# hzi-bifo/RiboDetector

Measured on AMD Instinct MI355X. Metric: reads/sec classified, 100 bp paired-end, higher is better.
Workload: dtype f16x3-split (f32 accumulate); 1 GPU; BASELINE configs[2]: paired-end 100 bp, --ensure rrna, 1048576 pairs/step/GPU x 49 steps (51.4 M total); pinned host bytes -> H2D -> kernels -> labels D2H (SURVEY 8d region ii); read_len=100, ensure=rrna, kernel_variant=mfma_f16x3_t32, parallelism=reads sharded x1, label gather to rank 0, rccl_ranks=1, forced_dist=False, prefix_k=12

## Files before the change

include/ribodetector_amd.h:

```cpp
#ifndef RIBODETECTOR_AMD_H
#define RIBODETECTOR_AMD_H

#include <stddef.h>
#include <stdint.h>

#ifndef RD_API
#define RD_API __attribute__((visibility("default")))
#endif

#ifdef __cplusplus
extern "C" {
#endif

#define RD_OK 0
#define RD_E_INVALID (-1)
#define RD_E_HIP (-2)
#define RD_E_UNSUPPORTED (-3)
#define RD_E_WORKSPACE (-4)

#define RD_ENSURE_NONE 0
#define RD_ENSURE_RRNA 1
#define RD_ENSURE_NORRNA 2
#define RD_ENSURE_BOTH 3

// ... 30 lines not shown
RD_API int rd_sync_results(rd_model *m, void *stream);
RD_API int rd_refine(const rd_model *m, const uint8_t *arena, const int64_t *seq_off, const int32_t *seq_len, int64_t n,
              int32_t max_len, float *logits, uint8_t *labels, const float *mate_logits, float thresh, void *stream);

#define RD_PREFIX_K_MIN 4
#define RD_PREFIX_K_MAX 13
RD_API size_t rd_prefix_table_bytes(int32_t k);
RD_API size_t rd_prefix_scratch_bytes(int32_t k);
RD_API int rd_set_prefix_table(rd_model *m, int32_t k, void *table, size_t table_bytes, void *scratch, size_t scratch_bytes, void *stream);
RD_API int rd_prefix_k(const rd_model *m);

RD_API size_t rd_classify_workspace_bytes(int64_t n, int32_t max_len);

RD_API int rd_classify(const rd_model *m, const uint8_t *arena, const int64_t *seq_off, const int32_t *seq_len, int64_t n,
                int32_t max_len, float *logits, uint8_t *labels, void *workspace, size_t workspace_bytes, void *stream);

RD_API int rd_pair_fuse(const float *logits1, const float *logits2, int64_t n, int32_t ensure_mode, int8_t *pair_labels,
                 uint64_t *counts, void *stream);

RD_API int rd_count_labels(const uint8_t *labels, int64_t n, uint64_t *counts, void *stream);

RD_API int rd_encode_codes(const uint8_t *arena, const int64_t *seq_off, const int32_t *seq_len, int64_t n, int32_t max_len,
                    int32_t stride, uint8_t *codes, void *stream);

RD_API int rd_encode_onehot_padded(const uint8_t *arena, const int64_t *seq_off, const int32_t *seq_len, int64_t n,
                            int32_t max_len, float *onehot, void *stream);

RD_API int rd_pack_plan(const int32_t *seq_len, int64_t n, int32_t max_len, int64_t *sorted_idx, int64_t *unsorted_idx,
                 int64_t *batch_sizes, int64_t *total_steps, void *workspace, size_t workspace_bytes, void *stream);
RD_API int rd_pack_onehot(const uint8_t *arena, const int64_t *seq_off, const int32_t *seq_len, int64_t n, int32_t max_len,
// ... 121 lines not shown
```

ribodetector_amd/_native.py:

```python
import ctypes as C
import os

_HERE = os.path.dirname(os.path.abspath(__file__))
LIB_PATH = os.environ.get("RD_HIP_LIB") or os.path.join(_HERE, "csrc", "librd_hip.so")

ENSURE_MODES = {"none": 0, "rrna": 1, "norrna": 2, "both": 3}
SEMANTICS = {"packed": 0, "gpu": 0, "padded": 1, "cpu": 1}
PREFIX_K_MIN, PREFIX_K_MAX, PREFIX_K_AUTO = 4, 13, 12
VARIANTS = {"auto": 0, "mfma_f32": 1, "simple": 2, "mfma_f16x3_t32": 4}
DIAG_VARIANTS = {"mfma_f32_a0s0": 10, "mfma_f32_a1s0": 11, "mfma_f32_a0s1": 12, "mfma_f32_a1s1": 13,
                 "mfma_f32_diag_noew": 20, "mfma_f32_diag_nomfma": 21, "mfma_f32_diag_mfmaonly": 22, "mfma_f32_diag_mfmabar": 23}
if os.path.basename(LIB_PATH).startswith("librd_hip_diag"):
    VARIANTS = dict(VARIANTS, **DIAG_VARIANTS)

SYMBOLS = [
    "rd_model_create", "rd_model_destroy", "rd_set_variant", "rd_variant_available", "rd_set_semantics", "rd_set_refine", "rd_set_refine_async", "rd_sync_results", "rd_refine", "rd_prefix_table_bytes", "rd_prefix_scratch_bytes", "rd_set_prefix_table", "rd_prefix_k", "rd_classify_workspace_bytes", "rd_classify",
    "rd_pair_fuse", "rd_count_labels", "rd_encode_codes", "rd_encode_onehot_padded", "rd_pack_plan",
    "rd_pack_onehot", "rd_profile_enable", "rd_profile_read", "rd_last_error", "rd_version",
    "rd_gz_workspace_bytes", "rd_gz_out_bound", "rd_gz_compress_selected", "rd_gz_eof_block", "rd_gz_inflate_members",
    "rd_fastq_index_workspace_bytes", "rd_fastq_index", "rd_fastq_gather", "rd_fastq_sample", "rd_fastq_strip_mark", "rd_fasta_index_workspace_bytes", "rd_fasta_index", "rd_fasta_gather", "rd_fasta_sample", "rd_select_workspace_bytes", "rd_select_pack", "rd_stream_create", "rd_stream_destroy", "rd_copy_bytes", "rd_gz_stream_workspace_bytes", "rd_gz_stream_inflate",
    "rd_gz_range_workspace_bytes", "rd_gz_range_decode", "rd_gz_range_resolve_workspace_bytes", "rd_gz_range_resolve",
    "rd_report_workspace_bytes", "rd_report_out_bound", "rd_report_format",
    "rd_pair_split", "rd_pair_expand_labels",
]
LABEL_SKIP = 2


class RdWeights(C.Structure):
    _fields_ = [(n, C.POINTER(C.c_float)) for n in
                ("w_ih", "w_hh", "b_ih", "b_hh", "w_ih_r", "w_hh_r", "b_ih_r", "b_hh_r", "w_out", "b_out")] + \
               [("input_size", C.c_int32), ("hidden_size", C.c_int32), ("num_classes", C.c_int32)]
# ... 21 lines not shown
    L.rd_variant_available.argtypes = [C.c_int]
    L.rd_set_semantics.argtypes = [vp, C.c_int]
    L.rd_set_refine.argtypes = [vp, C.c_float]
    L.rd_set_refine_async.argtypes = [vp, C.c_int]
    L.rd_sync_results.argtypes = [vp, vp]
    L.rd_refine.argtypes = [vp, vp, vp, vp, i64, i32, vp, vp, vp, C.c_float, vp]
    L.rd_prefix_table_bytes.argtypes = [i32]
    L.rd_prefix_table_bytes.restype = sz
    L.rd_prefix_scratch_bytes.argtypes = [i32]
    L.rd_prefix_scratch_bytes.restype = sz
    L.rd_set_prefix_table.argtypes = [vp, i32, vp, sz, vp, sz, vp]
    L.rd_prefix_k.argtypes = [vp]
    L.rd_classify_workspace_bytes.argtypes = [i64, i32]
    L.rd_classify_workspace_bytes.restype = sz
    L.rd_classify.argtypes = [vp, vp, vp, vp, i64, i32, vp, vp, vp, sz, vp]
    L.rd_pair_fuse.argtypes = [vp, vp, i64, i32, vp, vp, vp]
    L.rd_count_labels.argtypes = [vp, i64, vp, vp]
    L.rd_encode_codes.argtypes = [vp, vp, vp, i64, i32, i32, vp, vp]
    L.rd_encode_onehot_padded.argtypes = [vp, vp, vp, i64, i32, vp, vp]
    L.rd_pack_plan.argtypes = [vp, i64, i32, vp, vp, vp, vp, vp, sz, vp]
    L.rd_pack_onehot.argtypes = [vp, vp, vp, i64, i32, vp, vp, vp, vp]
    L.rd_gz_workspace_bytes.argtypes = [i64, i64]
    L.rd_gz_workspace_bytes.restype = sz
    L.rd_gz_out_bound.argtypes = [i64]
    L.rd_gz_out_bound.restype = sz
    L.rd_gz_compress_selected.argtypes = [vp, i64, vp, vp, i64, i32, vp, sz, vp, vp, sz, vp]
    L.rd_gz_eof_block.argtypes = [vp, sz]
    L.rd_gz_inflate_members.argtypes = [vp, i64, vp, i64, vp, i64, vp, vp]
    L.rd_fastq_index_workspace_bytes.argtypes = [i64]
    L.rd_fastq_index_workspace_bytes.restype = sz
# ... 132 lines not shown
```

ribodetector_amd/csrc/rd_kernels.hip:

```cpp
#include <stdlib.h>
#include "rd_common.hpp"
#include "rd_prep.hpp"
#include "rd_recurrence.hpp"
#include "rd_sort.hpp"
#include "rd_lstm_f32.hpp"
#include "rd_lstm_t32.hpp"
#include "rd_refine.hpp"
#include "rd_encode.hpp"
#include "rd_deflate.hpp"
#include "rd_inflate_dev.hpp"
#include "rd_inflate_stream.hpp"
#include "rd_fastq_index.hpp"
#include "rd_fasta_index.hpp"
#include "rd_report.hpp"
#include "rd_pairs.hpp"

extern "C" {

const char *rd_last_error(void) { return g_err; }
const char *rd_version(void) { return "ribodetector_amd 0.1.0 (gfx950)"; }

int rd_model_create(const rd_weights *w, int device, rd_model **out) {
    if (!w || !out) RD_FAIL(RD_E_INVALID, "rd_model_create: null argument");
    if (w->input_size != 4 || w->hidden_size != HID || w->num_classes != 2)
// ... 284 lines not shown
        m->prof_launches_accum += 1;
    }
    m->prof_count = 0;
    return RD_OK;
}

int rd_profile_read(rd_model *m, int64_t *launches, double *total_ms) {
    if (!m) RD_FAIL(RD_E_INVALID, "rd_profile_read: null model");
    int rc = rd_profile_drain(m);
    if (rc) return rc;
    if (launches) *launches = m->prof_launches_accum;
    if (total_ms) *total_ms = m->prof_ms_accum;
    return RD_OK;
}

int rd_classify(const rd_model *cm, const uint8_t *arena, const int64_t *seq_off, const int32_t *seq_len, int64_t n,
                int32_t max_len, float *logits, uint8_t *labels, void *workspace, size_t workspace_bytes, void *stream) {
    rd_model *m = const_cast<rd_model *>(cm);
    if (!m || !logits) RD_FAIL(RD_E_INVALID, "rd_classify: null model or logits");
    if (n < 0 || n > 0x7fffffffLL) RD_FAIL(RD_E_INVALID, "rd_classify: n=%lld out of range", (long long)n);
    if (max_len < 1 || max_len > MAX_LEN_LIMIT) RD_FAIL(RD_E_INVALID, "rd_classify: max_len=%d out of range [1,%d]", max_len, MAX_LEN_LIMIT);
    if (n == 0) return RD_OK;
    if (!arena || !seq_off || !seq_len || !workspace) RD_FAIL(RD_E_INVALID, "rd_classify: null input pointer");
    hipStream_t st = (hipStream_t)stream;
    const SortPlan sp = sort_plan(n, max_len);
    if (workspace_bytes < sp.total) RD_FAIL(RD_E_WORKSPACE, "workspace too small: %zu < %zu", workspace_bytes, sp.total);
    bool deferred = false;
    int join_after_launch = -1;
    if (m->refine_async && m->refine_thresh > 0.0f) {
        hipStreamCaptureStatus cap = hipStreamCaptureStatusNone;
        (void)hipStreamIsCapturing(st, &cap);
        deferred = cap == hipStreamCaptureStatusNone;
    }
    if (deferred) {
        bool clash = false;
        for (int x = 0; x < 2 && !clash; ++x)
            for (int k = 0; k < m->q_npend[x] && !clash; ++k) {
                const auto &pd = m->q_pend[x][k];
                const char *lo = (const char *)pd.p[3], *la = (const char *)pd.p[4];
                clash = (m->semantics == RD_SEM_PADDED && pd.max_len != max_len) ||
                        arena == pd.p[0] || seq_off == pd.p[1] || seq_len == pd.p[2] ||
                        ((const char *)logits < lo + 8 * pd.n && lo < (const char *)logits + 8 * n) ||
                        (labels && la && (const char *)labels < la + pd.n && la < (const char *)labels + n);
            }
        if (clash) { int rc0 = rd_sync_results(m, stream); if (rc0) return rc0; }
        if (m->q_calls >= m->refine_async) {
            const int old = m->q_cur;
            int rc0 = rd_async_flush(m, st, old);
            if (rc0) return rc0;
            m->q_cur ^= 1;
            m->q_calls = 0;
            rc0 = rd_async_join(m, st, m->q_cur);
            if (rc0) return rc0;
            join_after_launch = old;
        }
        int rc1 = rd_async_acquire(m, st, m->q_cur);
        if (rc1) return rc1;
    }
    if (m->semantics == RD_SEM_PADDED && m->rev_tab_len != max_len) {
        hipLaunchKernelGGL(rd_revtab_kernel, dim3(1), dim3(512), 0, st, m->d, max_len);
        m->rev_tab_len = max_len;
    }
    int32_t *steps = nullptr, *order = nullptr, *pfx = nullptr;
    const int pk = m->variant == m->ptab_variant ? m->prefix_k : 0;
    int rc = run_steps_and_buckets(arena, seq_off, seq_len, n, max_len, m->semantics, workspace, workspace_bytes, steps, order, pk, pfx, st);
    if (rc) return rc;
    ReadBatch rb{arena, seq_off, seq_len, steps, order, n, max_len, m->semantics, m->d.rev_tab, pk > 0 ? m->ptab : m->d.zero_row, pfx, pk,
                 deferred ? rd_queue(m, m->q_cur) : RefineQueue{nullptr, nullptr, 0}, m->refine_thresh};
    hipEvent_t *ev = nullptr;
    if (m->prof_enabled) {
        if (m->prof_count == 512) { rc = rd_profile_drain(m); if (rc) return rc; }
        ev = &m->prof_ev[2 * m->prof_count];
        for (int i = 0; i < 2; ++i)
            if (!ev[i]) RD_HIP(hipEventCreate(&ev[i]));
        RD_HIP(hipEventRecord(ev[0], st));
    }
    if (m->variant == RD_VARIANT_SIMPLE) {
        const int64_t nwg = (n + SB - 1) / SB;
        hipLaunchKernelGGL(rd_lstm_simple_kernel, dim3((unsigned)nwg), dim3(512), 0, st, m->d, rb, logits, labels);
    } else {
        const int64_t nwg = (n + BT - 1) / BT;
        const dim3 grid((unsigned)nwg), blk(256);
        switch (m->variant) {
// ... 14 lines not shown
    }
    RD_HIP(hipGetLastError());
    if (ev) { RD_HIP(hipEventRecord(ev[1], st)); m->prof_count++; }
    if (join_after_launch >= 0) {
        rc = rd_async_join(m, st, join_after_launch);
        if (rc) return rc;
    }
    if (m->refine_thresh > 0.0f) {
        if (!deferred) return rd_refine_launch(m, rb, logits, labels, nullptr, m->refine_thresh, st);
        auto &pd = m->q_pend[m->q_cur][m->q_npend[m->q_cur]++];
        pd.p[0] = arena; pd.p[1] = seq_off; pd.p[2] = seq_len; pd.p[3] = logits; pd.p[4] = labels;
        pd.n = n; pd.max_len = max_len; pd.sem = m->semantics; pd.thresh = m->refine_thresh;
        m->q_calls++;
    }
    return RD_OK;
}

int rd_pair_fuse(const float *logits1, const float *logits2, int64_t n, int32_t ensure_mode, int8_t *pair_labels,
                 uint64_t *counts, void *stream) {
    if (n < 0 || ensure_mode < 0 || ensure_mode > 3) RD_FAIL(RD_E_INVALID, "rd_pair_fuse: bad n or ensure_mode");
    if (n == 0) return RD_OK;
    if (!logits1 || !logits2 || !pair_labels) RD_FAIL(RD_E_INVALID, "rd_pair_fuse: null pointer");
    int64_t nb = (n + 2047) / 2048;
    if (nb > 1024) nb = 1024;
    const bool vec = (((uintptr_t)logits1 | (uintptr_t)logits2) & 15) == 0 && ((uintptr_t)pair_labels & 1) == 0;
    if (vec)
        hipLaunchKernelGGL(rd_pair_fuse_kernel<true>, dim3((unsigned)nb), dim3(256), 0, (hipStream_t)stream, (const float2 *)logits1,
                           (const float2 *)logits2, n, ensure_mode, pair_labels, counts);
    else
        hipLaunchKernelGGL(rd_pair_fuse_kernel<false>, dim3((unsigned)nb), dim3(256), 0, (hipStream_t)stream, (const float2 *)logits1,
// ... 559 lines not shown
```

ribodetector_amd/csrc/rd_lstm_f32.hpp:

```cpp
#pragma once
#include "rd_recurrence.hpp"

namespace {

struct __attribute__((aligned(16))) LstmSmem {
    float Hs[NT][16][HSTR];
    float Hl[NT][16][HSTR];
    f32x4 cA[NT][256];
    f32x4 cB[NT][256];
    f32x4 lut[5][4][16][2];
    float wout[2][HID];
    float dummy[256];
    uint8_t codes[2][TC][BT];
    int T[BT];
    int Lr[BT];
    long long off[BT];
    int orig[BT];
    int k0[BT];
    int prow[BT];
    int tmax;
};

__device__ __forceinline__ void rd_f32_load_h(LstmSmem &S, const uint8_t *ptab, int read) {
    const int piece = threadIdx.x & 3;
// ... 37 lines not shown
template <int ACT>
__device__ __forceinline__ float act_tanh(float x) {
    if (ACT == 0) return rd_tanh(x);
    return __builtin_fmaf(-2.0f, __builtin_amdgcn_rcpf(1.0f + __builtin_amdgcn_exp2f(x * 2.88539008177792681f)), 1.0f);
}

template <int ACT, int SCHED, int DIAG = 0, bool BUILD = false>
__global__ __launch_bounds__(256, 1) void rd_lstm_mfma_f32_kernel(DevModel d, ReadBatch rb, float *__restrict__ logits,
                                                                  uint8_t *__restrict__ labels) {
    __shared__ LstmSmem S;
    const int tid = threadIdx.x, lane = tid & 63;
    const int wave = __builtin_amdgcn_readfirstlane(tid >> 6);
    const int q = lane >> 4, l15 = lane & 15;

    const int nz = BUILD ? 0 : (rb.pk > 0 ? 1 << (2 * rb.pk) : 0);
    if (tid < BT) {
        const int64_t g = (int64_t)blockIdx.x * BT + tid;
        int T = 0, lr = 0, orig = -1, k0 = 0, prow = nz;
        long long off = 0;
        if (BUILD) {
            if (g < rb.n) { orig = (int)g; T = 1; lr = 1; if (rb.pk > 1) prow = (int)(g >> 2); }
        } else if (g < rb.n) {
            orig = rb.order ? rb.order[g] : (int)g;
            T = rd_T(rb.steps, orig, rb.max_len);
            lr = rd_T(rb.len, orig, rb.max_len);
            off = rb.off[orig];
            if (rb.pfx) {
                prow = rb.pfx[orig];
                if (prow != nz) { k0 = rb.pk; lr -= k0; off += k0; }
            }
        }
        S.T[tid] = T; S.Lr[tid] = lr; S.off[tid] = off; S.orig[tid] = orig; S.k0[tid] = k0; S.prow[tid] = prow;
    }
    if (tid == 0) S.tmax = 0;
    for (int i = tid; i < NT * 16 * HSTR; i += 256) (&S.Hl[0][0][0])[i] = 0.0f;
    for (int i = tid; i < 5 * G4; i += 256) {
        const int c = i & 7, l = (i >> 3) & 15, w = (i >> 7) & 3, code = i >> 9;
// ... 185 lines not shown
        }
    } else {
        rd_fc_epilogue(
            BT, [&](int row, int u) { return S.Hl[row >> 4][row & 15][u]; }, S.T, S.Lr, S.off, S.orig, &S.wout[0][0], d, rb, logits, labels,
            S.k0);
    }
}

constexpr int SB = 8;
__global__ __launch_bounds__(512) void rd_lstm_simple_kernel(DevModel d, ReadBatch rb, float *__restrict__ logits,
                                                             uint8_t *__restrict__ labels) {
    __shared__ float h[SB][HID], c[SB][HID], hl[SB][HID], g[SB][G4], s_wout[2 * HID];
    __shared__ int T[SB], Lr[SB], orig[SB], tmax_s;
    __shared__ long long off[SB];
    const int tid = threadIdx.x;
    if (tid < SB) {
        const int64_t gi = (int64_t)blockIdx.x * SB + tid;
        int Ti = 0, li = 0, o = -1;
        long long of = 0;
        if (gi < rb.n) { o = rb.order ? rb.order[gi] : (int)gi; Ti = rd_T(rb.steps, o, rb.max_len); li = rd_T(rb.len, o, rb.max_len); of = rb.off[o]; }
        T[tid] = Ti; Lr[tid] = li; orig[tid] = o; off[tid] = of;
    }
    if (tid == 0) tmax_s = 0;
    for (int i = tid; i < SB * HID; i += 512) { (&h[0][0])[i] = 0; (&c[0][0])[i] = 0; (&hl[0][0])[i] = 0; }
    if (tid < 256) s_wout[tid] = d.w_out[(tid >> 7) * 256 + (tid & 127)];
    __syncthreads();
    if (tid < SB) atomicMax(&tmax_s, T[tid]);
    __syncthreads();
    const int tmax = tmax_s;
    for (int t = 0; t < tmax; ++t) {
        float a[SB];
#pragma unroll
        for (int r = 0; r < SB; ++r) {
            int code = 4;
            if (t < Lr[r]) code = rd_code(rb.arena[off[r] + t]);
// ... 27 lines not shown
```

ribodetector_amd/csrc/rd_lstm_t32.hpp:

```cpp
#pragma once
#include "rd_recurrence.hpp"

namespace {

typedef float f32x16 __attribute__((ext_vector_type(16)));
typedef _Float16 f16x4 __attribute__((ext_vector_type(4)));
typedef float f32x2 __attribute__((ext_vector_type(2)));

constexpr int CSTR = TC16 + 4;
struct __attribute__((aligned(16))) Lstm16bSmem {
    f32x4 lut[4][2][4][4][6];
    _Float16 H1s[2][32][H16STR];
    _Float16 H2[2][32][H16STR];
    float Hl[64][HSTR];
    f32x4 dummy[256];
    float wout[2][HID];
    uint8_t codes[2][64][CSTR];
    int T[64];
    int Lr[64];
    long long off[64];
    int orig[64];
    int k0[64];
    u32x4 st_h[128][8];
    f32x4 st_c[4][256];
// ... 210 lines not shown
    c.last = (tEW == S.T[TP * 32 + j] - 1);
    c.any_last = __builtin_amdgcn_ballot_w64(c.last) != 0;
    rd_tail_rowtiles<TP, 0>(S, R, accP, c);
    __syncthreads();
}

template <bool BUILD>
__global__ __launch_bounds__(256, 1) void rd_lstm_mfma_f16x3_t32_kernel(DevModel d, ReadBatch rb, float *__restrict__ logits,
                                                                        uint8_t *__restrict__ labels) {
    __shared__ Lstm16bSmem S;
    const int tid = threadIdx.x, lane = tid & 63;
    const int wave = __builtin_amdgcn_readfirstlane(tid >> 6);
    const int half = lane >> 5, j = lane & 31;

    const int row = tid >> 2, piece = tid & 3;
    const int64_t g = (int64_t)blockIdx.x * 64 + row;
    const bool valid = g < rb.n;
    const int nz = BUILD ? 0 : (rb.pk > 0 ? 1 << (2 * rb.pk) : 0);
    const int64_t gc0 = (int64_t)blockIdx.x * 64 + j, gc1 = gc0 + 32;
    const bool use_pfx = !BUILD && rb.pfx != nullptr;
    int orig = -1, oc0 = -1, oc1 = -1;
    if (valid) orig = (!BUILD && rb.order) ? rb.order[g] : (int)g;
    if (use_pfx) {
        if (gc0 < rb.n) oc0 = rb.order ? rb.order[gc0] : (int)gc0;
        if (gc1 < rb.n) oc1 = rb.order ? rb.order[gc1] : (int)gc1;
    }
    f32x4 lut_v[3];
    {
        const f32x4 *src = reinterpret_cast<const f32x4 *>(d.lut_t32);
#pragma unroll
        for (int k = 0; k < 3; ++k) lut_v[k] = src[tid + 256 * k];
    }
    const float wout_v = d.w_out[(tid >> 7) * 256 + (tid & 127)];
    f16x8 W1[4][8], W2[4][8];
    const uint4 *wp = reinterpret_cast<const uint4 *>(d.wpack16b) + (size_t)wave * (2 * 4 * 8 * 64) + lane;
    auto load_row_tile = [&](auto a_c) {
        constexpr int a = decltype(a_c)::value;
        uint4 x[2][8];
#pragma unroll
        for (int hl = 0; hl < 2; ++hl)
// ... 142 lines not shown
```

ribodetector_amd/csrc/rd_recurrence.hpp:

```cpp
#pragma once
#include "rd_common.hpp"

namespace {

struct RefineEntry {
    const uint8_t *bases;
    float *logits;
    uint8_t *label;
    int32_t lr;
    int32_t max_len;
    int32_t sem;
    int32_t pad_;
};
struct RefineQueue {
    RefineEntry *e;
    uint32_t *count;
    uint32_t cap;
};

struct ReadBatch {
    const uint8_t *arena;
    const int64_t *off;
    const int32_t *len;
    const int32_t *steps;
    const int32_t *order;
    int64_t n;
    int max_len;
    int sem;
    const float *rev_tab;
    const uint8_t *ptab;
    const int32_t *pfx;
    int pk;
    RefineQueue rq;
    float rthresh;
};
constexpr int PFX_ROW = 1024;

template <typename HL>
__device__ __forceinline__ void rd_fc_epilogue(int nrows, HL hl, const int *Trow, const int *Lrow, const long long *offrow,
                                               const int *origrow, const float *s_wout, const DevModel &d, const ReadBatch &rb,
                                               float *logits, uint8_t *labels, const int *k0row = nullptr) {
    const int tid = threadIdx.x;
    if (tid < 2 * nrows) {
        const int row = tid >> 1, k = tid & 1;
        float s = d.b_out[k];
        for (int u = 0; u < HID; ++u) s = __builtin_fmaf(s_wout[k * HID + u], hl(row, u), s);
        const int T = Trow[row];
        if (rb.sem == RD_SEM_PADDED && T > 0) {
            const int pos = T - 1;
            const int code = pos < Lrow[row] ? rd_code(rb.arena[offrow[row] + pos]) : 4;
// ... 28 lines not shown
```

ribodetector_amd/csrc/rd_sort.hpp:

```cpp
#pragma once
#include "rd_common.hpp"

namespace {

constexpr int SORT_BLOCK = 256;
constexpr int SORT_ITEMS = 2048;


__global__ void rd_len_hist_kernel(const int32_t *__restrict__ len, int64_t n, int max_len, int nblk,
                                   uint32_t *__restrict__ hist) {
    extern __shared__ uint32_t sh[];
    for (int i = threadIdx.x; i <= max_len; i += blockDim.x) sh[i] = 0;
    __syncthreads();
    int64_t base = (int64_t)blockIdx.x * SORT_ITEMS;
    for (int k = threadIdx.x; k < SORT_ITEMS; k += blockDim.x) {
        int64_t i = base + k;
        if (i < n) atomicAdd(&sh[rd_T(len, i, max_len)], 1u);
    }
    __syncthreads();
    for (int i = threadIdx.x; i <= max_len; i += blockDim.x) hist[(size_t)i * nblk + blockIdx.x] = sh[i];
}

__global__ __launch_bounds__(SORT_BLOCK) void rd_len_rowscan_kernel(uint32_t *__restrict__ hist, int nblk, uint32_t *__restrict__ row_total) {
    __shared__ uint32_t part[SORT_BLOCK];
// ... 108 lines not shown
    const unsigned long long m = __ballot(valid);
    if (!m) return 0;
    const int lane = threadIdx.x & 63, first = __ffsll((long long)m) - 1;
    const int T0 = __shfl(T, first);
    if (__all(!valid || T == T0)) {
        uint32_t base = 0;
        if (lane == first) base = atomicAdd(&bins[T0], (uint32_t)__popcll(m));
        return __shfl(base, first) + (uint32_t)__popcll(m & ((1ull << lane) - 1));
    }
    return valid ? atomicAdd(&bins[T], 1u) : 0;
}

__global__ __launch_bounds__(256) void rd_steps_kernel(const uint8_t *__restrict__ arena, const int64_t *__restrict__ off,
                                                       const int32_t *__restrict__ len, int64_t n, int max_len, int sem,
                                                       int32_t *__restrict__ steps, uint32_t *__restrict__ ghist, int pk,
                                                       int32_t *__restrict__ pfx) {
    extern __shared__ uint32_t sh_bins[];
    for (int i = threadIdx.x; i <= max_len; i += 256) sh_bins[i] = 0;
    __syncthreads();
    for (int64_t base = (int64_t)blockIdx.x * 256; base < n; base += (int64_t)gridDim.x * 256) {
        const int64_t i = base + threadIdx.x;
        const bool valid = i < n;
        int T = 0;
        if (valid) {
            const int lr = rd_T(len, i, max_len);
            T = lr;
            if (sem == RD_SEM_PADDED) {
                const uint8_t *p = arena + off[i];
                int pos = lr - 1;
                while (pos >= 0 && rd_code(p[pos]) == 4) --pos;
                T = pos >= 0 ? pos + 1 : max_len;
            }
            if (pk > 0) {
                int prow = 1 << (2 * pk);
                if (T > pk && lr >= pk) {
                    const uint8_t *p = arena + off[i];
                    u32x4 raw = {0u, 0u, 0u, 0u};
                    if (lr >= 16) __builtin_memcpy(&raw, p, 16);
// ... 7 lines not shown
                    }
                    if (ok) { prow = (int)idx; T -= pk; }
                }
                pfx[i] = prow;
            }
            steps[i] = T;
        }
        rd_bin_add(sh_bins, T, valid);
    }
    __syncthreads();
    for (int i = threadIdx.x; i <= max_len; i += 256)
        if (sh_bins[i]) atomicAdd(&ghist[i], sh_bins[i]);
}

__global__ __launch_bounds__(256) void rd_bucket_scan_kernel(const uint32_t *__restrict__ ghist, int max_len,
                                                             uint32_t *__restrict__ cursor) {
    __shared__ uint32_t part[256];
    const int tid = threadIdx.x, nb = max_len + 1, per = (nb + 255) / 256;
    uint32_t s = 0;
    for (int k = 0; k < per; ++k) {
        const int e = tid * per + k;
        if (e < nb) s += ghist[max_len - e];
    }
    part[tid] = s;
    __syncthreads();
    for (int d = 1; d < 256; d <<= 1) {
        const uint32_t v = tid >= d ? part[tid - d] : 0;
        __syncthreads();
        part[tid] += v;
        __syncthreads();
    }
    uint32_t run = part[tid] - s;
    for (int k = 0; k < per; ++k) {
        const int e = tid * per + k;
        if (e < nb) {
            cursor[max_len - e] = run;
            run += ghist[max_len - e];
        }
    }
}

constexpr int BK_ITEMS = 2048;
__global__ __launch_bounds__(256) void rd_bucket_scatter_kernel(const int32_t *__restrict__ steps, int64_t n, int max_len,
                                                                uint32_t *__restrict__ cursor, int32_t *__restrict__ order) {
    extern __shared__ uint32_t sh_bins[];
    for (int64_t b0 = (int64_t)blockIdx.x * BK_ITEMS; b0 < n; b0 += (int64_t)gridDim.x * BK_ITEMS) {
        __syncthreads();
        for (int i = threadIdx.x; i <= max_len; i += 256) sh_bins[i] = 0;
        __syncthreads();
        int Tk[BK_ITEMS / 256];
        uint32_t rk[BK_ITEMS / 256];
#pragma unroll
        for (int k = 0; k < BK_ITEMS / 256; ++k) {
            const int64_t i = b0 + k * 256 + threadIdx.x;
            const bool valid = i < n;
            const int T = valid ? steps[i] : 0;
            rk[k] = rd_bin_add(sh_bins, T, valid);
            Tk[k] = valid ? T : -1;
        }
        __syncthreads();
        for (int i = threadIdx.x; i <= max_len; i += 256) {
            const uint32_t c = sh_bins[i];
            if (c) sh_bins[i] = atomicAdd(&cursor[i], c);
        }
        __syncthreads();
#pragma unroll
        for (int k = 0; k < BK_ITEMS / 256; ++k)
            if (Tk[k] >= 0) order[sh_bins[Tk[k]] + rk[k]] = (int32_t)(b0 + k * 256 + threadIdx.x);
    }
}

inline size_t align_up(size_t x, size_t a) { return (x + a - 1) / a * a; }

// ... 26 lines not shown
    order = (int32_t *)(w + p.hist_bytes);
    len_start = (int64_t *)(w + p.hist_bytes + p.order_bytes);
    const size_t sh = (size_t)(max_len + 1) * sizeof(uint32_t);
    hipLaunchKernelGGL(rd_len_hist_kernel, dim3(p.nblk), dim3(SORT_BLOCK), sh, st, seq_len, n, max_len, p.nblk, hist);
    uint32_t *row_total = (uint32_t *)(len_start + (max_len + 1));
    hipLaunchKernelGGL(rd_len_rowscan_kernel, dim3(max_len + 1), dim3(SORT_BLOCK), 0, st, hist, p.nblk, row_total);
    hipLaunchKernelGGL(rd_len_rowstart_kernel, dim3(1), dim3(SORT_BLOCK), 0, st, row_total, max_len, len_start, batch_sizes, total_steps);
    hipLaunchKernelGGL(rd_len_rowadd_kernel, dim3(max_len + 1), dim3(SORT_BLOCK), 0, st, hist, p.nblk, len_start);
    hipLaunchKernelGGL(rd_len_scatter_kernel, dim3(p.nblk), dim3(SORT_BLOCK), sh, st, seq_len, n, max_len, p.nblk, hist, order,
                       sorted_idx, unsorted_idx);
    RD_HIP(hipGetLastError());
    return RD_OK;
}

int run_steps_and_buckets(const uint8_t *arena, const int64_t *seq_off, const int32_t *seq_len, int64_t n, int max_len, int sem,
                          void *workspace, size_t wbytes, int32_t *&steps, int32_t *&order, int pk, int32_t *&pfx, hipStream_t st) {
    SortPlan p = sort_plan(n, max_len);
    if (wbytes < p.total) RD_FAIL(RD_E_WORKSPACE, "workspace too small: %zu < %zu", wbytes, p.total);
    char *w = (char *)workspace;
    uint32_t *ghist = (uint32_t *)w;
    order = (int32_t *)(w + p.hist_bytes);
    uint32_t *cursor = (uint32_t *)(w + p.hist_bytes + p.order_bytes);
    steps = (int32_t *)(w + p.total - p.pfx_bytes - p.steps_bytes);
    pfx = pk > 0 ? (int32_t *)(w + p.total - p.pfx_bytes) : nullptr;
    const size_t sh = (size_t)(max_len + 1) * sizeof(uint32_t);
    RD_HIP(hipMemsetAsync(ghist, 0, sh, st));
    int64_t nb = (n + 255) / 256;
    const int64_t nb_max = pk > 0 ? 2048 : 256;
    if (nb > nb_max) nb = nb_max;
    hipLaunchKernelGGL(rd_steps_kernel, dim3((unsigned)nb), dim3(256), sh, st, arena, seq_off, seq_len, n, max_len, sem, steps, ghist, pk, pfx);
    hipLaunchKernelGGL(rd_bucket_scan_kernel, dim3(1), dim3(256), 0, st, ghist, max_len, cursor);
    int64_t nbs = (n + BK_ITEMS - 1) / BK_ITEMS;
    if (nbs > 256) nbs = 256;
    hipLaunchKernelGGL(rd_bucket_scatter_kernel, dim3((unsigned)nbs), dim3(256), sh, st, steps, n, max_len, cursor, order);
    RD_HIP(hipGetLastError());
    return RD_OK;
}

}
```

ribodetector_amd/detect.py:

```python
#!/usr/bin/env python3
import argparse
import functools
import math
import os
import threading
import time
import queue
from argparse import RawTextHelpFormatter
from typing import NamedTuple, Optional

import numpy as np
import torch
import torch.distributed as dist

from . import __version__
from . import _native as _native_mod
from . import dist as rdist
from . import gz as _gzmod
from .data_loader import device_reader as dr
from .data_loader import fastx_parser as fx
from .model import model as module_arch
from .parse_config import ConfigParser

cd = os.path.dirname(os.path.abspath(__file__))
# ... 130 lines not shown
        self.logger = config.get_logger('predict', 1, self.args.log if int(os.environ.get('RANK', '0')) == 0 else None)
        log_level = log_level or os.environ.get('RD_LOG_LEVEL')
        import logging
        self.logger.setLevel(getattr(logging, str(log_level).upper()) if log_level else logging.NOTSET)
        self.chunk_size = self.args.chunk_size
        self.thread_cpu_s = {}
        self.rank, self.world, self.local_rank = 0, 1, 0
        self.multi = False
        self._arenas = []
        self._part_files = []
        self.sharded_parse = False
        self._shared = None
        self._chunk_reads = None
        self._use_device = None
        self._report = None
        self.interleaved = bool(getattr(args, 'interleaved', False))
        self.mate_check = not getattr(args, 'no_mate_check', False)
        self._pairs = None
        self._install_cleanup()

    @property
    def gathers_labels(self):
        return not self.sharded_parse and self.multi

    def cleanup(self):
        self._close_arenas()
        for f in self._part_files:
            try:
                os.remove(f)
            except OSError:
# ... 167 lines not shown
            bounds = rdist.shard_bounds(n, self.world, work)
        lo, hi = (0, n) if bounds is None else (bounds[self.rank], bounds[self.rank + 1])
        cs = self._copy_stream
        cur = torch.cuda.current_stream(self.device)
        on_dev = isinstance(chunks[0], dr.DeviceChunk)
        pairs = None
        if self.interleaved:
            dev_in, pairs = self._split_pairs(chunks[0], lo, hi, on_dev)
        elif on_dev:
            dev_in = [c.dev[:3] for c in chunks]
            for c in chunks:
                cur.wait_event(c.ready)
        else:
            dev_in = [self._to_device(c, lo, hi, cs) for c in chunks]
            cur.wait_stream(cs)
        outs = [self.model.classify_bytes(a, o, l, self.len, want_labels=not self.is_paired) for a, o, l in dev_in]
        main_done = torch.cuda.Event()
        main_done.record(cur)
        post = self._post_stream
        with torch.cuda.stream(post):
            post.wait_event(main_done)
            self.model.sync_results()
            if self.is_paired and self.args.ensure == 'none' and self.refine_band > 0:
                for k, (a, o, l) in enumerate(dev_in):
                    self.model.refine(a, o, l, self.len, outs[k][0], outs[k][1], outs[1 - k][0], thresh=self.refine_band)
            if self.is_paired:
                labels = module_arch.pair_fuse(outs[0][0], outs[1][0], self.args.ensure)
            else:
                labels = outs[0][1].view(torch.int8)
            host = None if self.gathers_labels else _pinned(labels)
            pieces = self._select_chunk(chunks, dev_in, labels, lo, hi, on_dev, pairs)
            if self._report is not None:
                pieces[REPORT] = self._report_chunk(chunks, dev_in, outs, labels, lo, hi, pairs)
            finish = None
            if self.gathers_labels:
                _, finish = rdist.gather_labels(labels, n, dst=0, bounds=bounds, async_op=True)
            done = _native_mod.new_event()
            done.record(post)
        return {"n": n, "bounds": bounds, "labels": labels, "host": host, "finish": finish, "done": done, "keep": (dev_in, outs),
                "pieces": pieces, "pairs": pairs, "chunk": chunks[0], "totals": [c.total for c in chunks] if on_dev else ()}
# ... 383 lines not shown
                files[-1][2].write_text(hdr.ctypes.data, hdr.size)
        return files

    def _device_outputs(self, out_files):
        self._gz_files, self._gz_seq = [], 0
        if self.gzip_on_device:
            self._gz_files = self.gz_output_files(self.output, self.rrna, self.is_paired, self.args.ensure)
        self._out_files = out_files
        if any(self._device_parse(p) for p in self.input):
            self._sel = _gzmod.DeviceSelect(self.device)
        self._pairs, self._pair_seq = (_gzmod.DevicePairSplit(self.device) if self.interleaved else None), 0
        rep_path = getattr(self.args, 'read_report', None)
        self._report = _gzmod.DeviceReport(self.device) if rep_path else None
        self._rep_gz = bool(rep_path) and self.gzip_on_device and rep_path.endswith('gz')
        self._rep_seq = 0
        if self._gz_files or self._rep_gz:
            self._gz = _gzmod.DeviceGzip(self.device)

    def _in_flight(self, stream):
        prev = None
        for chunks in stream:
            t0 = time.perf_counter()
            self._mark("chunk_of_%d_read" % len(chunks[0].seq_len), t0)
            tk = self.submit_chunk(chunks)
            self._mark("submitted")
            self._stage_s["classify"] += time.perf_counter() - t0
            if prev is not None:
                yield prev
            prev = (chunks, tk)
        if prev is not None:
            yield prev

# ... 167 lines not shown
    config = ConfigParser.from_json(config_file)
    seq_pred = Predictor(config, args, log_level=log_level)
    try:
        t0 = time.perf_counter()
        seq_pred.load_model()
        t1 = time.perf_counter()
        seq_pred.detect()
        t2 = time.perf_counter()
        fc = getattr(seq_pred, "_first_chunk", None)
        steady = None
        if fc is not None and seq_pred.num_read > fc[1] and t2 > fc[0]:
            steady = (2 if seq_pred.is_paired else 1) * (seq_pred.num_read - fc[1]) / (t2 - fc[0])
        seq_pred.timing = {"load_model_s": t1 - t0, "detect_s": t2 - t1, "prefix_k": seq_pred.model.prefix_k,
                           "reads_per_s_after_first_chunk": steady, "ingest": getattr(seq_pred, "ingest", None),
                           "gz_ranges_s": getattr(seq_pred, "gz_shard_s", None), "pinned_cpus": getattr(seq_pred, "pinned_cpus", None),
                           "first_chunks_timeline": getattr(seq_pred, "_timeline", None), "run_started_at": getattr(seq_pred, "_t_run", None)}
        if os.environ.get("RD_TIMING_OUT"):
            import json
            with open("%s.rank%d" % (os.environ["RD_TIMING_OUT"], seq_pred.rank), "w") as fh:
                json.dump(dict(seq_pred.timing, rank=seq_pred.rank, world=seq_pred.world, num_read=seq_pred.num_read,
                               thread_cpu_s=seq_pred.thread_cpu_s, process_cpu_s=time.process_time(), main_thread_s=getattr(seq_pred, "_stage_s", None),
                               phases_s=getattr(seq_pred, "phases_s", None)), fh, default=str)
    except BaseException:
        seq_pred.cleanup()
        if seq_pred.multi:
            import sys
            import traceback
            traceback.print_exc()
            sys.stdout.flush()
            sys.stderr.flush()
            os._exit(1)
# ... 7 lines not shown
```

ribodetector_amd/model/model.py:

```python
import contextlib
import ctypes as C
import logging
import os

import numpy as np
import torch
from torch.nn.utils.rnn import PackedSequence

from .. import _native as N

log = logging.getLogger("ribodetector_amd")


@contextlib.contextmanager
def _device_lock(device):
    import fcntl
    import tempfile
    try:
        uid = str(torch.cuda.get_device_properties(device).uuid)
    except Exception:
        uid = "dev%d" % (device.index if device.index is not None else torch.cuda.current_device())
    path = os.path.join(tempfile.gettempdir(), "rd_prefix_%s.lock" % "".join(ch for ch in uid if ch.isalnum() or ch in "-_"))
    fd = os.open(path, os.O_CREAT | os.O_RDWR, 0o666)
    try:
# ... 225 lines not shown
    def refine_pairs(self, arena, offsets, lens, max_len, logits, mate_logits, labels=None, thresh=None):
        return self.refine(arena, offsets, lens, max_len, logits, labels, mate_logits, thresh)

    def __del__(self):
        try:
            self._destroy()
        except Exception:
            pass

    def _workspace(self, n, max_len):
        need = int(N.lib().rd_classify_workspace_bytes(n, max_len))
        if self._ws is None or self._ws.numel() < need or self._ws.device != self.device:
            self._ws = torch.empty(max(need, 1 << 16), dtype=torch.uint8, device=self.device)
        return self._ws

    def classify_bytes(self, arena, offsets, lens, max_len, want_labels=True, logits=None, labels=None):
        if self._handle is None:
            raise RuntimeError("SeqModel: call .to('cuda') before inference")
        n = int(lens.numel())
        for t, dt, nm in ((arena, torch.uint8, "arena"), (offsets, torch.int64, "offsets"), (lens, torch.int32, "lens")):
            if t.dtype != dt or not t.is_cuda or not t.is_contiguous():
                raise TypeError("classify_bytes: %s must be a contiguous %s CUDA tensor" % (nm, dt))
        if offsets.numel() < n:
            raise ValueError("classify_bytes: offsets shorter than lens")
        if logits is None:
            logits = torch.empty((n, 2), dtype=torch.float32, device=self.device)
        if want_labels and labels is None:
            labels = torch.empty((n,), dtype=torch.uint8, device=self.device)
        ws = self._workspace(n, max_len)
        with torch.cuda.device(self.device):
            return self._classify_launch(arena, offsets, lens, n, max_len, logits, labels, want_labels, ws)

    def _classify_launch(self, arena, offsets, lens, n, max_len, logits, labels, want_labels, ws):
        N.check(N.lib().rd_classify(self._handle, N.ptr(arena), N.ptr(offsets), N.ptr(lens), n, int(max_len), N.ptr(logits),
                                    N.ptr(labels if want_labels else None), N.ptr(ws), ws.numel(), N.stream_ptr(self.device)),
                "rd_classify")
        return logits, (labels if want_labels else None)

    def forward2(self, x):
        if not torch.is_tensor(x) or x.dim() != 3 or x.shape[2] != 4:
            raise TypeError("SeqModel.forward2 expects a padded Tensor [B, L, 4]; got %s" % (tuple(x.shape) if torch.is_tensor(x) else type(x).__name__))
        if self._handle is None:
            raise RuntimeError("SeqModel: call .to('cuda') before inference")
        dev = self.device
        data = x.to(dev, non_blocking=True)
        B, L = int(data.shape[0]), int(data.shape[1])
        if B == 0:
            return torch.empty((0, 2), dtype=torch.float32, device=dev)
        rs, mx = data.sum(2), data.max(2)
        ok = ((rs == 1) & (mx.values == 1)) | ((rs == 0) & (data.abs().sum(2) == 0))
        if not bool(ok.all()):
# ... 83 lines not shown
```

Baseline: 35.50 million reads/s.

## Skip LSTM on mate 2 when mate 1 already decides the pair under ensure

Under ensure rrna/norrna, mate 1's logits are passed into mate 2's classify. Reads whose mate is confidently labelled with the deciding class copy the mate logits, get steps=-1, and drop out of the length-bucket sort. A device-side live count lets the LSTM kernels exit early for blocks past the live reads. This avoids recurrent compute for pairs whose fused label is already fixed, at the cost of a serial dependency between mate 1 and mate 2 and extra async-queue join logic.

```diff
diff --git a/include/ribodetector_amd.h b/include/ribodetector_amd.h
--- a/include/ribodetector_amd.h
+++ b/include/ribodetector_amd.h
@@ -68,6 +68,10 @@
 
 RD_API int rd_classify(const rd_model *m, const uint8_t *arena, const int64_t *seq_off, const int32_t *seq_len, int64_t n,
                 int32_t max_len, float *logits, uint8_t *labels, void *workspace, size_t workspace_bytes, void *stream);
+
+RD_API int rd_classify_mate(const rd_model *m, const uint8_t *arena, const int64_t *seq_off, const int32_t *seq_len, int64_t n,
+                int32_t max_len, float *logits, uint8_t *labels, const float *mate_logits, int32_t ensure_mode, void *workspace,
+                size_t workspace_bytes, void *stream);
 
 RD_API int rd_pair_fuse(const float *logits1, const float *logits2, int64_t n, int32_t ensure_mode, int8_t *pair_labels,
                  uint64_t *counts, void *stream);
diff --git a/ribodetector_amd/_native.py b/ribodetector_amd/_native.py
--- a/ribodetector_amd/_native.py
+++ b/ribodetector_amd/_native.py
@@ -14,7 +14,7 @@
     VARIANTS = dict(VARIANTS, **DIAG_VARIANTS)
 
 SYMBOLS = [
-    "rd_model_create", "rd_model_destroy", "rd_set_variant", "rd_variant_available", "rd_set_semantics", "rd_set_refine", "rd_set_refine_async", "rd_sync_results", "rd_refine", "rd_prefix_table_bytes", "rd_prefix_scratch_bytes", "rd_set_prefix_table", "rd_prefix_k", "rd_classify_workspace_bytes", "rd_classify",
+    "rd_model_create", "rd_model_destroy", "rd_set_variant", "rd_variant_available", "rd_set_semantics", "rd_set_refine", "rd_set_refine_async", "rd_sync_results", "rd_refine", "rd_prefix_table_bytes", "rd_prefix_scratch_bytes", "rd_set_prefix_table", "rd_prefix_k", "rd_classify_workspace_bytes", "rd_classify", "rd_classify_mate",
     "rd_pair_fuse", "rd_count_labels", "rd_encode_codes", "rd_encode_onehot_padded", "rd_pack_plan",
     "rd_pack_onehot", "rd_profile_enable", "rd_profile_read", "rd_last_error", "rd_version",
     "rd_gz_workspace_bytes", "rd_gz_out_bound", "rd_gz_compress_selected", "rd_gz_eof_block", "rd_gz_inflate_members",
@@ -66,6 +66,7 @@
     L.rd_classify_workspace_bytes.argtypes = [i64, i32]
     L.rd_classify_workspace_bytes.restype = sz
     L.rd_classify.argtypes = [vp, vp, vp, vp, i64, i32, vp, vp, vp, sz, vp]
+    L.rd_classify_mate.argtypes = [vp, vp, vp, vp, i64, i32, vp, vp, vp, i32, vp, sz, vp]
     L.rd_pair_fuse.argtypes = [vp, vp, i64, i32, vp, vp, vp]
     L.rd_count_labels.argtypes = [vp, i64, vp, vp]
     L.rd_encode_codes.argtypes = [vp, vp, vp, i64, i32, i32, vp, vp]
diff --git a/ribodetector_amd/csrc/rd_kernels.hip b/ribodetector_amd/csrc/rd_kernels.hip
--- a/ribodetector_amd/csrc/rd_kernels.hip
+++ b/ribodetector_amd/csrc/rd_kernels.hip
@@ -322,8 +322,9 @@
     return RD_OK;
 }
 
-int rd_classify(const rd_model *cm, const uint8_t *arena, const int64_t *seq_off, const int32_t *seq_len, int64_t n,
-                int32_t max_len, float *logits, uint8_t *labels, void *workspace, size_t workspace_bytes, void *stream) {
+static int rd_classify_impl(const rd_model *cm, const uint8_t *arena, const int64_t *seq_off, const int32_t *seq_len, int64_t n,
+                            int32_t max_len, float *logits, uint8_t *labels, const float *mate_logits, int ensure_mode, void *workspace,
+                            size_t workspace_bytes, void *stream) {
     rd_model *m = const_cast<rd_model *>(cm);
     if (!m || !logits) RD_FAIL(RD_E_INVALID, "rd_classify: null model or logits");
     if (n < 0 || n > 0x7fffffffLL) RD_FAIL(RD_E_INVALID, "rd_classify: n=%lld out of range", (long long)n);
@@ -333,7 +334,7 @@
     hipStream_t st = (hipStream_t)stream;
     const SortPlan sp = sort_plan(n, max_len);
     if (workspace_bytes < sp.total) RD_FAIL(RD_E_WORKSPACE, "workspace too small: %zu < %zu", workspace_bytes, sp.total);
-    bool deferred = false;
+    bool deferred = false, mate_join = false;
     int join_after_launch = -1;
     if (m->refine_async && m->refine_thresh > 0.0f) {
         hipStreamCaptureStatus cap = hipStreamCaptureStatusNone;
@@ -352,6 +353,16 @@
                         (labels && la && (const char *)labels < la + pd.n && la < (const char *)labels + n);
             }
         if (clash) { int rc0 = rd_sync_results(m, stream); if (rc0) return rc0; }
+        if (mate_logits) {
+            const char *ml = (const char *)mate_logits;
+            for (int x = 0; x < 2; ++x)
+                for (int k = 0; k < m->q_npend[x]; ++k) {
+                    const auto &pd = m->q_pend[x][k];
+                    const char *lo = (const char *)pd.p[3];
+                    if (ml < lo + 8 * pd.n && lo < ml + 8 * n && (m->q_flushing[x] || (x == m->q_cur && m->q_calls >= m->refine_async)))
+                        mate_join = true;
+                }
+        }
         if (m->q_calls >= m->refine_async) {
             const int old = m->q_cur;
             int rc0 = rd_async_flush(m, st, old);
@@ -362,6 +373,8 @@
             if (rc0) return rc0;
             join_after_launch = old;
         }
+        if (mate_join)
+            for (int x = 0; x < 2; ++x) { int rc0 = rd_async_join(m, st, x); if (rc0) return rc0; }
         int rc1 = rd_async_acquire(m, st, m->q_cur);
         if (rc1) return rc1;
     }
@@ -371,10 +384,12 @@
     }
     int32_t *steps = nullptr, *order = nullptr, *pfx = nullptr;
     const int pk = m->variant == m->ptab_variant ? m->prefix_k : 0;
-    int rc = run_steps_and_buckets(arena, seq_off, seq_len, n, max_len, m->semantics, workspace, workspace_bytes, steps, order, pk, pfx, st);
+    const uint32_t *live = nullptr;
+    int rc = run_steps_and_buckets(arena, seq_off, seq_len, n, max_len, m->semantics, workspace, workspace_bytes, steps, order, pk, pfx, live,
+                                   mate_logits, ensure_mode, m->refine_thresh, logits, labels, st);
     if (rc) return rc;
     ReadBatch rb{arena, seq_off, seq_len, steps, order, n, max_len, m->semantics, m->d.rev_tab, pk > 0 ? m->ptab : m->d.zero_row, pfx, pk,
-                 deferred ? rd_queue(m, m->q_cur) : RefineQueue{nullptr, nullptr, 0}, m->refine_thresh};
+                 deferred ? rd_queue(m, m->q_cur) : RefineQueue{nullptr, nullptr, 0}, m->refine_thresh, live};
     hipEvent_t *ev = nullptr;
     if (m->prof_enabled) {
         if (m->prof_count == 512) { rc = rd_profile_drain(m); if (rc) return rc; }
@@ -419,6 +434,23 @@
         m->q_calls++;
     }
     return RD_OK;
+}
+
+int rd_classify(const rd_model *m, const uint8_t *arena, const int64_t *seq_off, const int32_t *seq_len, int64_t n, int32_t max_len,
+                float *logits, uint8_t *labels, void *workspace, size_t workspace_bytes, void *stream) {
+    return rd_classify_impl(m, arena, seq_off, seq_len, n, max_len, logits, labels, nullptr, RD_ENSURE_NONE, workspace, workspace_bytes, stream);
+}
+
+int rd_classify_mate(const rd_model *m, const uint8_t *arena, const int64_t *seq_off, const int32_t *seq_len, int64_t n, int32_t max_len,
+                     float *logits, uint8_t *labels, const float *mate_logits, int32_t ensure_mode, void *workspace,
+                     size_t workspace_bytes, void *stream) {
+    if (ensure_mode != RD_ENSURE_RRNA && ensure_mode != RD_ENSURE_NORRNA)
+        RD_FAIL(RD_E_INVALID, "rd_classify_mate: ensure_mode %d: only RD_ENSURE_RRNA and RD_ENSURE_NORRNA let one mate decide a pair", ensure_mode);
+    if (n > 0 && (!mate_logits || !logits)) RD_FAIL(RD_E_INVALID, "rd_classify_mate: null logits or mate_logits");
+    if (n > 0 && (const char *)mate_logits < (const char *)logits + 8 * n && (const char *)logits < (const char *)mate_logits + 8 * n)
+        RD_FAIL(RD_E_INVALID, "rd_classify_mate: logits and mate_logits overlap");
+    if ((((uintptr_t)logits | (uintptr_t)mate_logits) & 7)) RD_FAIL(RD_E_INVALID, "rd_classify_mate: logits and mate_logits must be 8-byte aligned");
+    return rd_classify_impl(m, arena, seq_off, seq_len, n, max_len, logits, labels, mate_logits, ensure_mode, workspace, workspace_bytes, stream);
 }
 
 int rd_pair_fuse(const float *logits1, const float *logits2, int64_t n, int32_t ensure_mode, int8_t *pair_labels,
diff --git a/ribodetector_amd/csrc/rd_lstm_f32.hpp b/ribodetector_amd/csrc/rd_lstm_f32.hpp
--- a/ribodetector_amd/csrc/rd_lstm_f32.hpp
+++ b/ribodetector_amd/csrc/rd_lstm_f32.hpp
@@ -75,13 +75,15 @@
     const int q = lane >> 4, l15 = lane & 15;
 
     const int nz = BUILD ? 0 : (rb.pk > 0 ? 1 << (2 * rb.pk) : 0);
+    const int64_t nlive = BUILD ? rb.n : rd_live(rb);
+    if (!BUILD && (int64_t)blockIdx.x * BT >= nlive) return;
     if (tid < BT) {
         const int64_t g = (int64_t)blockIdx.x * BT + tid;
         int T = 0, lr = 0, orig = -1, k0 = 0, prow = nz;
         long long off = 0;
         if (BUILD) {
             if (g < rb.n) { orig = (int)g; T = 1; lr = 1; if (rb.pk > 1) prow = (int)(g >> 2); }
-        } else if (g < rb.n) {
+        } else if (g < nlive) {
             orig = rb.order ? rb.order[g] : (int)g;
             T = rd_T(rb.steps, orig, rb.max_len);
             lr = rd_T(rb.len, orig, rb.max_len);
@@ -297,11 +299,13 @@
     __shared__ int T[SB], Lr[SB], orig[SB], tmax_s;
     __shared__ long long off[SB];
     const int tid = threadIdx.x;
+    const int64_t nlive = rd_live(rb);
+    if ((int64_t)blockIdx.x * SB >= nlive) return;
     if (tid < SB) {
         const int64_t gi = (int64_t)blockIdx.x * SB + tid;
         int Ti = 0, li = 0, o = -1;
         long long of = 0;
-        if (gi < rb.n) { o = rb.order ? rb.order[gi] : (int)gi; Ti = rd_T(rb.steps, o, rb.max_len); li = rd_T(rb.len, o, rb.max_len); of = rb.off[o]; }
+        if (gi < nlive) { o = rb.order ? rb.order[gi] : (int)gi; Ti = rd_T(rb.steps, o, rb.max_len); li = rd_T(rb.len, o, rb.max_len); of = rb.off[o]; }
         T[tid] = Ti; Lr[tid] = li; orig[tid] = o; off[tid] = of;
     }
     if (tid == 0) tmax_s = 0;
diff --git a/ribodetector_amd/csrc/rd_lstm_t32.hpp b/ribodetector_amd/csrc/rd_lstm_t32.hpp
--- a/ribodetector_amd/csrc/rd_lstm_t32.hpp
+++ b/ribodetector_amd/csrc/rd_lstm_t32.hpp
@@ -248,16 +248,18 @@
     const int half = lane >> 5, j = lane & 31;
 
     const int row = tid >> 2, piece = tid & 3;
+    const int64_t nlive = BUILD ? rb.n : rd_live(rb);
+    if (!BUILD && (int64_t)blockIdx.x * 64 >= nlive) return;
     const int64_t g = (int64_t)blockIdx.x * 64 + row;
-    const bool valid = g < rb.n;
+    const bool valid = g < nlive;
     const int nz = BUILD ? 0 : (rb.pk > 0 ? 1 << (2 * rb.pk) : 0);
     const int64_t gc0 = (int64_t)blockIdx.x * 64 + j, gc1 = gc0 + 32;
     const bool use_pfx = !BUILD && rb.pfx != nullptr;
     int orig = -1, oc0 = -1, oc1 = -1;
     if (valid) orig = (!BUILD && rb.order) ? rb.order[g] : (int)g;
     if (use_pfx) {
-        if (gc0 < rb.n) oc0 = rb.order ? rb.order[gc0] : (int)gc0;
-        if (gc1 < rb.n) oc1 = rb.order ? rb.order[gc1] : (int)gc1;
+        if (gc0 < nlive) oc0 = rb.order ? rb.order[gc0] : (int)gc0;
+        if (gc1 < nlive) oc1 = rb.order ? rb.order[gc1] : (int)gc1;
     }
     f32x4 lut_v[3];
     {
diff --git a/ribodetector_amd/csrc/rd_recurrence.hpp b/ribodetector_amd/csrc/rd_recurrence.hpp
--- a/ribodetector_amd/csrc/rd_recurrence.hpp
+++ b/ribodetector_amd/csrc/rd_recurrence.hpp
@@ -33,7 +33,10 @@
     int pk;
     RefineQueue rq;
     float rthresh;
+    const uint32_t *live;
 };
+
+__device__ __forceinline__ int64_t rd_live(const ReadBatch &rb) { return rb.live ? (int64_t)*rb.live : rb.n; }
 constexpr int PFX_ROW = 1024;
 
 template <typename HL>
diff --git a/ribodetector_amd/csrc/rd_sort.hpp b/ribodetector_amd/csrc/rd_sort.hpp
--- a/ribodetector_amd/csrc/rd_sort.hpp
+++ b/ribodetector_amd/csrc/rd_sort.hpp
@@ -146,14 +146,25 @@
 __global__ __launch_bounds__(256) void rd_steps_kernel(const uint8_t *__restrict__ arena, const int64_t *__restrict__ off,
                                                        const int32_t *__restrict__ len, int64_t n, int max_len, int sem,
                                                        int32_t *__restrict__ steps, uint32_t *__restrict__ ghist, int pk,
-                                                       int32_t *__restrict__ pfx) {
+                                                       int32_t *__restrict__ pfx, const float2 *__restrict__ mate, int ensure,
+                                                       float band, float2 *__restrict__ logits, uint8_t *__restrict__ labels) {
     extern __shared__ uint32_t sh_bins[];
     for (int i = threadIdx.x; i <= max_len; i += 256) sh_bins[i] = 0;
     __syncthreads();
     for (int64_t base = (int64_t)blockIdx.x * 256; base < n; base += (int64_t)gridDim.x * 256) {
         const int64_t i = base + threadIdx.x;
-        const bool valid = i < n;
+        bool valid = i < n;
         int T = 0;
+        if (valid && mate) {
+            const float2 m = mate[i];
+            const int lab = m.y > m.x;
+            if (fabsf(m.y - m.x) > band && lab == (ensure == RD_ENSURE_NORRNA)) {
+                logits[i] = m;
+                if (labels) labels[i] = (uint8_t)lab;
+                steps[i] = -1;
+                valid = false;
+            }
+        }
         if (valid) {
             const int lr = rd_T(len, i, max_len);
             T = lr;
@@ -191,7 +202,7 @@
 }
 
 __global__ __launch_bounds__(256) void rd_bucket_scan_kernel(const uint32_t *__restrict__ ghist, int max_len,
-                                                             uint32_t *__restrict__ cursor) {
+                                                             uint32_t *__restrict__ cursor, uint32_t *__restrict__ live) {
     __shared__ uint32_t part[256];
     const int tid = threadIdx.x, nb = max_len + 1, per = (nb + 255) / 256;
     uint32_t s = 0;
@@ -207,6 +218,7 @@
         part[tid] += v;
         __syncthreads();
     }
+    if (tid == 255) *live = part[255];
     uint32_t run = part[tid] - s;
     for (int k = 0; k < per; ++k) {
         const int e = tid * per + k;
@@ -230,10 +242,9 @@
 #pragma unroll
         for (int k = 0; k < BK_ITEMS / 256; ++k) {
             const int64_t i = b0 + k * 256 + threadIdx.x;
-            const bool valid = i < n;
-            const int T = valid ? steps[i] : 0;
-            rk[k] = rd_bin_add(sh_bins, T, valid);
-            Tk[k] = valid ? T : -1;
+            const int T = i < n ? steps[i] : -1;
+            rk[k] = rd_bin_add(sh_bins, T, T >= 0);
+            Tk[k] = T;
         }
         __syncthreads();
         for (int i = threadIdx.x; i <= max_len; i += 256) {
@@ -290,13 +301,16 @@
 }
 
 int run_steps_and_buckets(const uint8_t *arena, const int64_t *seq_off, const int32_t *seq_len, int64_t n, int max_len, int sem,
-                          void *workspace, size_t wbytes, int32_t *&steps, int32_t *&order, int pk, int32_t *&pfx, hipStream_t st) {
+                          void *workspace, size_t wbytes, int32_t *&steps, int32_t *&order, int pk, int32_t *&pfx, const uint32_t *&live,
+                          const float *mate_logits, int ensure, float band, float *logits, uint8_t *labels, hipStream_t st) {
     SortPlan p = sort_plan(n, max_len);
     if (wbytes < p.total) RD_FAIL(RD_E_WORKSPACE, "workspace too small: %zu < %zu", wbytes, p.total);
     char *w = (char *)workspace;
     uint32_t *ghist = (uint32_t *)w;
     order = (int32_t *)(w + p.hist_bytes);
     uint32_t *cursor = (uint32_t *)(w + p.hist_bytes + p.order_bytes);
+    uint32_t *nlive = cursor + (max_len + 1);
+    live = nlive;
     steps = (int32_t *)(w + p.total - p.pfx_bytes - p.steps_bytes);
     pfx = pk > 0 ? (int32_t *)(w + p.total - p.pfx_bytes) : nullptr;
     const size_t sh = (size_t)(max_len + 1) * sizeof(uint32_t);
@@ -304,8 +318,9 @@
     int64_t nb = (n + 255) / 256;
     const int64_t nb_max = pk > 0 ? 2048 : 256;
     if (nb > nb_max) nb = nb_max;
-    hipLaunchKernelGGL(rd_steps_kernel, dim3((unsigned)nb), dim3(256), sh, st, arena, seq_off, seq_len, n, max_len, sem, steps, ghist, pk, pfx);
-    hipLaunchKernelGGL(rd_bucket_scan_kernel, dim3(1), dim3(256), 0, st, ghist, max_len, cursor);
+    hipLaunchKernelGGL(rd_steps_kernel, dim3((unsigned)nb), dim3(256), sh, st, arena, seq_off, seq_len, n, max_len, sem, steps, ghist, pk, pfx,
+                       (const float2 *)mate_logits, ensure, band, (float2 *)logits, labels);
+    hipLaunchKernelGGL(rd_bucket_scan_kernel, dim3(1), dim3(256), 0, st, ghist, max_len, cursor, nlive);
     int64_t nbs = (n + BK_ITEMS - 1) / BK_ITEMS;
     if (nbs > 256) nbs = 256;
     hipLaunchKernelGGL(rd_bucket_scatter_kernel, dim3((unsigned)nbs), dim3(256), sh, st, steps, n, max_len, cursor, order);
diff --git a/ribodetector_amd/detect.py b/ribodetector_amd/detect.py
--- a/ribodetector_amd/detect.py
+++ b/ribodetector_amd/detect.py
@@ -168,6 +168,7 @@
         self._chunk_reads = None
         self._use_device = None
         self._report = None
+        self._mate_skip = False
         self.interleaved = bool(getattr(args, 'interleaved', False))
         self.mate_check = not getattr(args, 'no_mate_check', False)
         self._pairs = None
@@ -365,7 +366,11 @@
         else:
             dev_in = [self._to_device(c, lo, hi, cs) for c in chunks]
             cur.wait_stream(cs)
-        outs = [self.model.classify_bytes(a, o, l, self.len, want_labels=not self.is_paired) for a, o, l in dev_in]
+        outs = []
+        for k, (a, o, l) in enumerate(dev_in):
+            mate = outs[0][0] if k == 1 and self._mate_skip else None
+            outs.append(self.model.classify_bytes(a, o, l, self.len, want_labels=not self.is_paired, decided_by=mate,
+                                                  ensure=None if mate is None else self.args.ensure))
         main_done = torch.cuda.Event()
         main_done.record(cur)
         post = self._post_stream
@@ -375,6 +380,9 @@
             if self.is_paired and self.args.ensure == 'none' and self.refine_band > 0:
                 for k, (a, o, l) in enumerate(dev_in):
                     self.model.refine(a, o, l, self.len, outs[k][0], outs[k][1], outs[1 - k][0], thresh=self.refine_band)
+            if self._mate_skip:
+                self._mate_skipped += (outs[1][0].view(torch.int64) == outs[0][0].view(torch.int64)).sum()
+                self._mate_seen += hi - lo
             if self.is_paired:
                 labels = module_arch.pair_fuse(outs[0][0], outs[1][0], self.args.ensure)
             else:
@@ -788,8 +796,16 @@
         self._report = _gzmod.DeviceReport(self.device) if rep_path else None
         self._rep_gz = bool(rep_path) and self.gzip_on_device and rep_path.endswith('gz')
         self._rep_seq = 0
+        self._mate_skip = (self.is_paired and self.args.ensure in ('rrna', 'norrna') and self._report is None
+                           and os.environ.get("RD_MATE_SKIP", "1") != "0")
+        self._mate_skipped, self._mate_seen = torch.zeros((), dtype=torch.int64, device=self.device), 0
         if self._gz_files or self._rep_gz:
             self._gz = _gzmod.DeviceGzip(self.device)
+
+    def mate2_skipped_frac(self):
+        if not self._mate_skip or not self._mate_seen:
+            return None
+        return int(self._mate_skipped) / self._mate_seen
 
     def _in_flight(self, stream):
         prev = None
@@ -987,7 +1003,8 @@
         seq_pred.timing = {"load_model_s": t1 - t0, "detect_s": t2 - t1, "prefix_k": seq_pred.model.prefix_k,
                            "reads_per_s_after_first_chunk": steady, "ingest": getattr(seq_pred, "ingest", None),
                            "gz_ranges_s": getattr(seq_pred, "gz_shard_s", None), "pinned_cpus": getattr(seq_pred, "pinned_cpus", None),
-                           "first_chunks_timeline": getattr(seq_pred, "_timeline", None), "run_started_at": getattr(seq_pred, "_t_run", None)}
+                           "first_chunks_timeline": getattr(seq_pred, "_timeline", None), "run_started_at": getattr(seq_pred, "_t_run", None),
+                           "mate2_skipped_frac": seq_pred.mate2_skipped_frac()}
         if os.environ.get("RD_TIMING_OUT"):
             import json
             with open("%s.rank%d" % (os.environ["RD_TIMING_OUT"], seq_pred.rank), "w") as fh:
diff --git a/ribodetector_amd/model/model.py b/ribodetector_amd/model/model.py
--- a/ribodetector_amd/model/model.py
+++ b/ribodetector_amd/model/model.py
@@ -263,10 +263,19 @@
             self._ws = torch.empty(max(need, 1 << 16), dtype=torch.uint8, device=self.device)
         return self._ws
 
-    def classify_bytes(self, arena, offsets, lens, max_len, want_labels=True, logits=None, labels=None):
+    def classify_bytes(self, arena, offsets, lens, max_len, want_labels=True, logits=None, labels=None, decided_by=None, ensure=None):
+        n = int(lens.numel())
+        if (decided_by is None) != (ensure is None):
+            raise ValueError("classify_bytes: decided_by and ensure go together")
+        if decided_by is not None:
+            if ensure not in ("rrna", "norrna"):
+                raise ValueError("classify_bytes: a mate decides a pair only under ensure 'rrna' or 'norrna'; got %r" % (ensure,))
+            if not torch.is_tensor(decided_by) or decided_by.dtype != torch.float32 or not decided_by.is_cuda or not decided_by.is_contiguous():
+                raise TypeError("classify_bytes: decided_by must be a contiguous torch.float32 CUDA tensor")
+            if tuple(decided_by.shape) != (n, 2):
+                raise ValueError("classify_bytes: decided_by must have shape (%d, 2); got %s" % (n, tuple(decided_by.shape)))
         if self._handle is None:
             raise RuntimeError("SeqModel: call .to('cuda') before inference")
-        n = int(lens.numel())
         for t, dt, nm in ((arena, torch.uint8, "arena"), (offsets, torch.int64, "offsets"), (lens, torch.int32, "lens")):
             if t.dtype != dt or not t.is_cuda or not t.is_contiguous():
                 raise TypeError("classify_bytes: %s must be a contiguous %s CUDA tensor" % (nm, dt))
@@ -278,12 +287,17 @@
             labels = torch.empty((n,), dtype=torch.uint8, device=self.device)
         ws = self._workspace(n, max_len)
         with torch.cuda.device(self.device):
-            return self._classify_launch(arena, offsets, lens, n, max_len, logits, labels, want_labels, ws)
-
-    def _classify_launch(self, arena, offsets, lens, n, max_len, logits, labels, want_labels, ws):
-        N.check(N.lib().rd_classify(self._handle, N.ptr(arena), N.ptr(offsets), N.ptr(lens), n, int(max_len), N.ptr(logits),
-                                    N.ptr(labels if want_labels else None), N.ptr(ws), ws.numel(), N.stream_ptr(self.device)),
-                "rd_classify")
+            return self._classify_launch(arena, offsets, lens, n, max_len, logits, labels, want_labels, ws, decided_by, ensure)
+
+    def _classify_launch(self, arena, offsets, lens, n, max_len, logits, labels, want_labels, ws, decided_by=None, ensure=None):
+        if decided_by is None:
+            N.check(N.lib().rd_classify(self._handle, N.ptr(arena), N.ptr(offsets), N.ptr(lens), n, int(max_len), N.ptr(logits),
+                                        N.ptr(labels if want_labels else None), N.ptr(ws), ws.numel(), N.stream_ptr(self.device)),
+                    "rd_classify")
+        else:
+            N.check(N.lib().rd_classify_mate(self._handle, N.ptr(arena), N.ptr(offsets), N.ptr(lens), n, int(max_len), N.ptr(logits),
+                                             N.ptr(labels if want_labels else None), N.ptr(decided_by), N.ENSURE_MODES[ensure], N.ptr(ws),
+                                             ws.numel(), N.stream_ptr(self.device)), "rd_classify_mate")
         return logits, (labels if want_labels else None)
 
     def forward2(self, x):
```

Measured after the change: 35.41 million reads/s. No clear change (-0.2%).
